# razoumov/radiativeTransfer

Hardware: AMD Instinct MI355X
Metric: cell·dir·ν updates/sec per iteration, 256³ grid; achieved HBM GB/s vs peak (higher is better)
Workload: dtype f64

## Files before the change

### radiativetransfer_amd/csrc/ftte_api.cpp

```cpp
#include "ftte_context.h"

using namespace ftte;

namespace ftte {

std::string g_create_error;

int fail(ftte_ctx *c, int code, const std::string &msg)
{
    if (c) c->err = msg;
    else g_create_error = msg;
    return code;
}

int check_single(ftte_ctx *c)
{
    if (c && c->multi) return check_ready(c, false);
    return c ? FTTE_OK : FTTE_ERR_ARG;
}

}


extern "C" {
// ... 288 lines not shown
    if (c->multi) return multi_counter(c, name);
    if (!std::strcmp(name, "devices")) return 1;
    if (!std::strcmp(name, "grid_builds")) return c->n_grid_builds;
    if (!std::strcmp(name, "plan_builds")) return c->n_plan_builds;
    if (!std::strcmp(name, "forest_builds")) return c->n_forest_builds;
    if (!std::strcmp(name, "device_objects")) return g_device_objects.load();
    if (!std::strcmp(name, "population_slots")) return c->point.tables.slot_count();
    if (!std::strcmp(name, "expansion_exact_tests")) return c->chem.expansion_tests;
    if (!std::strcmp(name, "medium_abun2")) return c->gas.ready_with_abundance(c->ncell) ? 1 : 0;
    if (!std::strcmp(name, "catalogue_stars")) return c->catalogue.stars();
    if (!std::strcmp(name, "catalogue_sources")) return c->catalogue.sources();
    if (!std::strncmp(name, "catalogue_ns_", 13)) {
        static const char *const phase[4] = {"locate", "count", "scan", "emit"};
        for (int p = 0; p < 4; ++p)
            if (!std::strcmp(name + 13, phase[p])) return catalogue_phase_ns(c->catalogue, p);
        return -1;
    }
    if (!std::strcmp(name, "hybrid_boxes")) return c->hplan.boxes();
    if (!std::strcmp(name, "hybrid_passes")) return c->hplan.passes();
    if (!std::strcmp(name, "fine_block")) return c->hplan.fine_block();
    if (!std::strcmp(name, "brick_form")) return c->last_brick_form;
    if (!std::strcmp(name, "brick_dataflow")) return c->last_brick_dataflow;
    if (!std::strcmp(name, "brick_whole")) return c->last_brick_whole;
    if (!std::strcmp(name, "nu_deal")) return c->opt.launch.nu_deal;
    if (!std::strcmp(name, "brick_chunk")) return c->bplan.valid ? c->bplan.chunk : 0;
    if (!std::strcmp(name, "brick_queue_mix")) return (c->bplan.valid && c->bplan.persistent) ? c->bplan.key.queue_mix : -1;
    if (!std::strcmp(name, "brick_groups")) return c->bplan.valid ? (long long)c->bplan.groups.size() : 0;
    if (!std::strcmp(name, "brick_accumulators")) return c->bplan.valid ? c->bplan.nacc[0] + c->bplan.nacc[1] + c->bplan.nacc[2] : 0;
    if (!std::strcmp(name, "brick_accumulators_0")) return c->bplan.valid ? c->bplan.nacc[0] : 0;
    if (!std::strcmp(name, "brick_accumulators_1")) return c->bplan.valid ? c->bplan.nacc[1] : 0;
    if (!std::strcmp(name, "brick_accumulators_2")) return c->bplan.valid ? c->bplan.nacc[2] : 0;
    if (!std::strcmp(name, "brick_stages")) return c->bplan.valid ? c->bplan.nstages : 0;
    if (!std::strcmp(name, "merge_points")) return c->bplan.valid ? (long long)c->bplan.merge_stage.size() : 0;
    if (!std::strcmp(name, "merge_blocks")) return c->bplan.valid ? (long long)c->bplan.merge_blocks.size() : 0;
    if (!std::strncmp(name, "merge_stage_", 12) || !std::strncmp(name, "merge_final_", 12)) {
        char *end = nullptr;
        const long k = std::strtol(name + 12, &end, 10);
        if (!c->bplan.valid || end == name + 12 || *end || k < 0 || k >= (long)c->bplan.merge_stage.size()) return -1;
        return name[6] == 's' ? c->bplan.merge_stage[(size_t)k] : (long long)c->bplan.merge_off[(size_t)k + 1];
    }
    return -1;
}

int ftte_launch_count(const ftte_ctx *c) { return !c ? 0 : c->multi ? multi_first(c)->timing_used : c->timing_used; }

int ftte_launch_info(ftte_ctx *c, int idx, double *ms, int64_t *updates)
// ... 335 lines not shown
```

### radiativetransfer_amd/csrc/ftte_brick.hip

```cpp
#include <hip/hip_runtime.h>

#include "ftte_internal.h"
#include "ftte_kernels.h"
#include "ftte_math.h"

namespace ftte {

using gcbyte = const __attribute__((address_space(1))) char;
using gbyte = __attribute__((address_space(1))) char;
using gcdouble = const __attribute__((address_space(1))) double;
using gdouble = __attribute__((address_space(1))) double;

__device__ __forceinline__ int uniform(int x) { return __builtin_amdgcn_readfirstlane(x); }
__device__ __forceinline__ gcbyte *lane_address(gcbyte *base, unsigned offset) { asm volatile("" : "+s"(base)); return base + offset; }
__device__ __forceinline__ gbyte *lane_address(gbyte *base, unsigned offset) { asm volatile("" : "+s"(base)); return base + offset; }
__device__ __forceinline__ unsigned here(unsigned offset) { asm volatile("" : "+v"(offset)); return offset; }
__device__ __forceinline__ long here(long step) { asm volatile("" : "+s"(step)); return step; }

template <int ROWS, bool NT>
__device__ __forceinline__ void load_rows(double (&dst)[ROWS], gcbyte *row, unsigned off, long step, int nrows)
{
    if (nrows == ROWS) {
        off = here(off);
#pragma unroll
// ... 663 lines not shown
                for (int r = 0; r < H; ++r) {
                    if (r < nrows) {
                        if (accumulate && atomic_acc) (void)__builtin_amdgcn_global_atomic_fadd_f64((gdouble *)lane_address(jrow, off), Jacc[r]);
                        else __builtin_nontemporal_store(Jacc[r], (gdouble *)lane_address(jrow, off));
                    }
                    jrow += rstep;
                }
            }
        }
        __syncthreads();
    }

    if (has_i_out) {
        for (int q = 0; q < ndir; ++q) {
            int d = p0 + q;
            d = d >= ndir ? d - ndir : d;
            gdouble *f = (gdouble *)(G->dir[d].faces + fnu);
#pragma unroll
            for (int r = 0; r < H; ++r) f[i_out + (long)r * up] = q ? state[((q - 1) * H + r) * 64 + lane] : cur[r];
        }
    }
}

__global__ void xcc_census_kernel(unsigned *mask)
{
    unsigned xcc;
    asm volatile("s_getreg_b32 %0, hwreg(HW_REG_XCC_ID)" : "=s"(xcc));
    if (threadIdx.x == 0) atomicOr(mask, 1u << (xcc & 15u));
}

int launch_xcc_census(unsigned *mask_dev, hipStream_t stream)
{
    hipLaunchKernelGGL(xcc_census_kernel, dim3(4096), dim3(64), 0, stream, mask_dev);
    return hipGetLastError() == hipSuccess ? 0 : -2;
}

int launch_brick_pair(const BrickLaunch &L, int max_dirs, int waves, int lds_pad, hipStream_t stream)
{
    if (L.ntasks <= 0) return 0;
    if (max_dirs < 1 || max_dirs > kBrickMaxDirs || L.ticket != nullptr) return -1;
    const dim3 grid((unsigned)L.ntasks * (unsigned)L.nnu);
    const size_t lds = ((size_t)(max_dirs - 1) * kBrickRows * 64 + 2 * max_dirs * 64) * sizeof(double) + (size_t)lds_pad;
    if (L.emit == 1) hipLaunchKernelGGL((brick_pair_kernel<3, 1>), grid, dim3(128), lds, stream, L, max_dirs);
    else if (L.emit == 2) hipLaunchKernelGGL((brick_pair_kernel<4, 2>), grid, dim3(128), lds, stream, L, max_dirs);
    else if (L.emit) return -1;
    else switch (waves) {
    case 2: hipLaunchKernelGGL((brick_pair_kernel<2, 0>), grid, dim3(128), lds, stream, L, max_dirs); break;
    case 3: hipLaunchKernelGGL((brick_pair_kernel<3, 0>), grid, dim3(128), lds, stream, L, max_dirs); break;
    case 4: hipLaunchKernelGGL((brick_pair_kernel<4, 0>), grid, dim3(128), lds, stream, L, max_dirs); break;
    default: return -1;
    }
    return hipGetLastError() == hipSuccess ? 0 : -2;
}

bool brick_whole_form(const BrickLaunch &L, int waves, bool masked)
{
    return !masked && !L.emit && !L.ticket && !L.queue && waves == 4 && L.n % 64 == 0 && L.n % kBrickRows == 0 && !L.atomic_acc && !L.ablate;
}

int launch_brick(const BrickLaunch &L, int max_dirs, int waves, int lds_pad, hipStream_t stream, bool masked, int persistent)
{
    if (L.ntasks <= 0) return 0;
    if (max_dirs < 1 || max_dirs > kBrickMaxDirs) return -1;
    if (L.tiled && (L.emit || masked)) return -1;
    const dim3 grid((unsigned)L.ntasks * (unsigned)L.nnu);
    const size_t lds = (size_t)(max_dirs - 1) * kBrickRows * 64 * sizeof(double) + (size_t)lds_pad;
    const bool flow = L.ticket != nullptr;
    if (L.queue) {
        if (masked || L.emit || !flow || persistent < 1) return -1;
        hipLaunchKernelGGL((brick_kernel<4, 0, 2>), dim3((unsigned)persistent), dim3(64), lds, stream, L);
        return hipGetLastError() == hipSuccess ? 0 : -2;
    }
    if (masked && !flow && L.emit) {
        if (L.emit == 1) hipLaunchKernelGGL((brick_kernel<2, 1, 0, true>), grid, dim3(64), lds, stream, L);
        else hipLaunchKernelGGL((brick_kernel<3, 2, 0, true>), grid, dim3(64), lds, stream, L);
        return hipGetLastError() == hipSuccess ? 0 : -2;
    }
    if (masked) {
        if (flow) return -1;
        hipLaunchKernelGGL((brick_kernel<3, 0, 0, true>), grid, dim3(64), lds, stream, L);
        return hipGetLastError() == hipSuccess ? 0 : -2;
    }
    if (L.emit == 1 && !flow) hipLaunchKernelGGL((brick_kernel<3, 1, 0>), grid, dim3(64), lds, stream, L);
    else if (L.emit == 2 && !flow) hipLaunchKernelGGL((brick_kernel<3, 2, 0>), grid, dim3(64), lds, stream, L);
    else if (L.emit) return -1;
// ... 15 lines not shown
```

### radiativetransfer_amd/csrc/ftte_bricks.h

```cpp
#pragma once

#include <algorithm>
#include <cstdio>
#include <cstdlib>
#include <cstring>
#include <functional>
#include <string>
#include <vector>

#include "../../include/ftte.h"
#include "ftte_device.h"
#include "ftte_internal.h"

namespace ftte {

struct DirPlan {
    int izone = 0, layout = 0;
    double phi = 0, theta = 0, w = 0;
    int64_t org = 0;
    int si = 0, sv = 0, su = 0;
    int u_lo = 1, v_lo = 1, ntu = 0, ntv = 0;
    int du_mid = 0, dv_mid = 0;
    size_t layer_off = 0;
    int slot = 0;
};

struct BrickKey {
    int n = 0;
    double box = 0;
    int chunk = 0, gmax = 0, share = 0;
    int want_dataflow = 0, want_glanes = 0;
    int nnu = 0, xcc_count = 0, queue_mix = 0;
    bool operator==(const BrickKey &o) const
    {
        return n == o.n && box == o.box && chunk == o.chunk && gmax == o.gmax && share == o.share && want_dataflow == o.want_dataflow &&
               want_glanes == o.want_glanes && nnu == o.nnu && xcc_count == o.xcc_count && queue_mix == o.queue_mix;
    }
};

struct BrickOptions {
    int chunk = 0, group = 0;
    int share = 2, team = -1, lanes = 2;
    int dataflow = 0;
    int queue_mix = 0;

    int brick_form(int nnu, int emit_mode) const { return team >= 0 ? team : (((nnu <= 4 || emit_mode) && !dataflow) ? 2 : 0); }

    BrickKey resolve(int n, int nnu, int emit_mode) const
    {
        BrickKey k;
        const int form = brick_form(nnu, emit_mode);
        k.n = n;
        k.chunk = std::min(chunk > 0 ? chunk : (nnu >= 4 ? 16 : nnu >= 2 ? 8 : 4), n);
        k.gmax = group > 0 ? group : (nnu >= 2 || form == 2 ? 3 : 2);
        k.share = share;
        k.want_dataflow = (dataflow && n % 64 == 0 && n % kBrickRows == 0 && n % k.chunk == 0 && form == 0 && !emit_mode) ? 1 : 0;
        k.want_glanes = k.want_dataflow ? 1 : (nnu >= lanes ? 1 : lanes);
        return k;
    }
    void persistent(BrickKey &k, int nnu, int xcc_count) const
    {
        if (!k.want_dataflow || dataflow != 3 || xcc_count < 1 || xcc_count > kBrickQueues) return;
        k.want_dataflow = 3; k.nnu = nnu; k.xcc_count = xcc_count; k.queue_mix = queue_mix;
    }
    BrickKey resolve_hybrid(int n, int nnu) const
    {
        BrickKey k;
        k.n = n;
        k.chunk = std::min(chunk > 0 ? chunk : 4, n);
        k.gmax = group > 0 ? group : (nnu >= 2 ? 3 : 2);
        k.share = share;
        return k;
    }
};

struct BrickPlan {
    bool valid = false;
    long long id = 0;
    BrickKey key;
    std::vector<double> phi, theta, w;
    int n = 0, chunk = 0;
    std::vector<DirPlan> dirs;
    std::vector<LayerRec> layers;
    struct Group { int izone = 0, layout = 0, acc = 0, offset = 0, lane = 0; std::vector<int> dirs; };
    std::vector<Group> groups;
    std::vector<BrickTask> tasks;
    bool dataflow = false;
    std::vector<int32_t> deps;
    bool persistent = false;
    std::vector<uint32_t> queue;
    uint32_t qoff[kBrickQueues] = {}, qlen[kBrickQueues] = {};
    int64_t qload[kBrickQueues] = {};
    int ut = kBrickRows, uw = 0;
    int64_t uqface_off = 0;
    int nslot = 2;
    int glanes = 1, nstages = 0;
    std::vector<size_t> stage_off;
    int64_t updates = 0;
    int ntu = 0, ntv = 0, nti = 0, up = 0, vp = 0, max_dirs = 0;
    int64_t face_elems = 0, vface_off = 0, iface_off = 0;
    int nacc[3] = {0, 0, 0};
    int nmb = 0;
    std::vector<int32_t> merge_blocks;
    std::vector<int> merge_stage;
    std::vector<size_t> merge_off;
};

struct SubGridPlan {
    int n = 0;
// ... 26 lines not shown
public:
    T *get() const { return buf_; }
    operator T *() const { return get(); }
    void reset() { buf_.reset(); held_.clear(); }
    hipError_t send(const T *src, size_t count)
    {
        bool fresh = false;
        hipError_t e = buf_.reserve(count, &fresh);
        if (fresh || e != hipSuccess) held_.clear();
        const size_t bytes = sizeof(T) * count;
        if (e != hipSuccess || !bytes || (held_.size() == bytes && !std::memcmp(held_.data(), src, bytes))) return e;
        held_.clear();
        if ((e = hipMemcpy(buf_, src, bytes, hipMemcpyHostToDevice)) == hipSuccess) held_.assign((const char *)src, (const char *)src + bytes);
        return e;
    }
private:
    DeviceBuffer<T> buf_;
    std::vector<char> held_;
};

struct BrickTables {
    DeviceBuffer<LayerRec> layers; DeviceBuffer<BrickTask> tasks; Sent<BrickGroup> groups;
    DeviceBuffer<int32_t> deps, merge_blocks; DeviceBuffer<uint32_t> queue;
    bool holds(const BrickPlan &P) const { return held_ != 0 && held_ == P.id; }
    hipError_t upload(const BrickPlan &P)
    {
        if (holds(P)) return hipSuccess;
        held_ = 0;
        hipError_t e;
        if ((e = to_device(layers, P.layers)) != hipSuccess || (e = to_device(tasks, P.tasks)) != hipSuccess) return e;
        if (P.dataflow && !P.deps.empty() && (e = to_device(deps, P.deps)) != hipSuccess) return e;
        if (!P.merge_blocks.empty() && (e = to_device(merge_blocks, P.merge_blocks)) != hipSuccess) return e;
        if (P.persistent && !P.queue.empty() && (e = to_device(queue, P.queue)) != hipSuccess) return e;
        held_ = P.id;
        return hipSuccess;
    }
private:
    long long held_ = 0;
};

inline BrickLaunch brick_launch(const BrickPlan &P, const BrickTables &T, size_t task0, size_t task1, int nu0, int nu1, int64_t group_stride,
                                int64_t face_stride, const double *uvb, int emit)
{
    BrickLaunch L;
    std::memset(&L, 0, sizeof L);
    L.groups = T.groups; L.tasks = T.tasks + task0; L.uvb = uvb;
    L.group_stride = group_stride; L.face_stride = face_stride;
    L.vface_off = P.vface_off; L.iface_off = P.iface_off; L.uqface_off = P.uqface_off;
    L.n = P.n; L.ntasks = (int)(task1 - task0); L.nnu = nu1 - nu0; L.nu0 = nu0; L.chunk = P.chunk;
    L.up = P.up; L.vp = P.vp; L.uw = P.uw; L.ut = P.ut; L.nslot = P.nslot;
    L.emit = emit; L.math = kMath;
    return L;
}

struct AccList { const double *acc[3 * kMaxAcc]; int layout[3 * kMaxAcc]; int count = 0; };
inline AccList acc_list(const DeviceBuffer<double> (&set)[3][kMaxAcc], const int (&nacc)[3], const int (&frame)[3], size_t offset = 0)
// ... 87 lines not shown
```

### radiativetransfer_amd/csrc/ftte_context.h

```cpp
#pragma once

#include <hip/hip_runtime_api.h>

#include <algorithm>
#include <cmath>
#include <cstdio>
#include <cstring>
#include <functional>
#include <string>
#include <vector>

#include "../../include/ftte.h"
#include "ftte_amr.h"
#include "ftte_analysis.h"
#include "ftte_bricks.h"
#include "ftte_gas.h"
#include "ftte_geometry.h"
#include "ftte_host.h"
#include "ftte_hybrid.h"
#include "ftte_kernels.h"
#include "ftte_lambda.h"
#include "ftte_medium.h"
#include "ftte_options.h"
#include "ftte_point.h"
// ... 22 lines not shown
namespace ftte { struct Multi; }

struct ftte_ctx {
    ftte::Multi *multi = nullptr;
    int device = 0;
    Stream stream;
    std::string err;

    bool grid_set = false;
    int n = 0;
    int64_t ncell = 0;
    double box = 0;

    Options opt;

    int nnu = 0;
    MediumField kappa;

    int emit_mode = 0;
    MediumField emis;

    DeviceBuffer<double> acc[3][kMaxAcc];

    int last_brick_form = -1, last_brick_dataflow = -1, last_brick_whole = 0;
    std::vector<Stream> lane_stream;
    std::vector<Event> pipe_up;
    std::vector<Event> lane_done;
    Event ev_fork;
    BrickDataflow bflow;
    int xcc_count = -1;
    int8_t xcc_queue[16] = {};
    long long brick_plans = 0;
    BrickPlan bplan;
    BrickTables btables;
    DeviceBuffer<double> d_faces;

    Plan plan;
    DeviceBuffer<LayerRec> d_layers;
    DeviceBuffer<WorkItem> d_items;
    Sent<double> d_uvb;
    bool plan_uploaded = false;

    std::vector<LaunchTiming> timing;
    int timing_used = 0;

    AmrTree tree;
    DeviceTree dtree;
// ... 118 lines not shown
```

### radiativetransfer_amd/csrc/ftte_internal.h

```cpp
#pragma once
#include <cstdint>

#include "ftte_math.h"

namespace ftte {

enum RayClass : int {
    RC_ONE = 0,
    RC_TWO_U = 1,
    RC_TWO_V = 2,
    RC_THREE_U = 3,
    RC_THREE_V = 4,
    RC_THREE_U_SWAP = 5,
    RC_THREE_V_SWAP = 6
};

struct LayerRec {
    double dpath[3];
    int32_t info;
    int32_t drift;
};
static_assert(sizeof(LayerRec) == 32, "LayerRec must be 32 bytes");

struct DirRec {
// ... 41 lines not shown
    const LayerRec *layers;
    double *faces;
    double w;
    double pad;
};

struct BrickGroup {
    BrickDir dir[kBrickMaxDirs];
    const double *kappa;
    const double *emis;
    double *J;
    int64_t org;
    int32_t si, sv, su;
    int32_t ndir;
    int32_t bu, bv;
    int64_t bi;
};

struct BrickTask { int16_t group, tu, tv, ti; };
constexpr int kBrickAccumulate = 0x4000;
constexpr int kBrickTuMask = 0x3ff, kBrickLaneLoShift = 10, kBrickGroupMask = 0xff, kBrickLaneHiShift = 8;
constexpr int kBrickTvMask = 0x3ff, kBrickBoxShift = 10, kBrickBoxMask = 31;
static_assert(sizeof(BrickTask) == 8, "BrickTask must be 8 bytes");

struct BrickLaunch {
    const BrickGroup *groups;
    const BrickTask *tasks;
    const double *uvb;
    int64_t group_stride;
    int64_t face_stride;
    int64_t vface_off, iface_off;
    int64_t uqface_off;
    int32_t n, ntasks, nnu, chunk;
    int32_t nu0;
    int32_t emit;
    int32_t up, vp;
    int32_t nslot;
    int32_t uw, ut;
    uint32_t *ticket, *done, *error;
    const int32_t *deps;
    uint32_t epoch;
    int32_t through;
    int32_t tiled, ablate;
    const uint32_t *queue;
    uint32_t qoff[kBrickQueues], qlen[kBrickQueues];
    int8_t xcc_queue[16];
    int32_t atomic_acc;
    int32_t sub;
    int32_t deal;
    ftte_consts math;
};

constexpr unsigned kXcds = 8;
struct BrickWork { unsigned task, slot; };
FTTE_HD BrickWork brick_deal(unsigned work, unsigned nnu, unsigned deal)
{
    BrickWork W;
    W.task = work / nnu;
    W.slot = work - W.task * nnu;
    if (deal) {
        const unsigned low = nnu & (0u - nnu), g = low < kXcds ? low : kXcds;
        W.slot = (W.slot + W.task / (kXcds / g * deal)) % nnu;
    }
    return W;
}

constexpr int kAmrBatch = 96;

struct SegRec {
    int32_t seg;
    int32_t up, up2;
    int32_t at;
// ... 91 lines not shown
```

### radiativetransfer_amd/csrc/ftte_kernels.h

```cpp
#pragma once
#include <hip/hip_runtime_api.h>

#include "ftte_internal.h"

namespace ftte {

int launch_sweep(const LaunchRec &L, int rows, int waves, int stack, int nnu, int lds_pad, hipStream_t stream);
int launch_brick(const BrickLaunch &L, int max_dirs, int waves, int lds_pad, hipStream_t stream, bool masked = false, int persistent = 0);
bool brick_whole_form(const BrickLaunch &L, int waves, bool masked = false);
int launch_xcc_census(unsigned *mask_dev, hipStream_t stream);
int launch_brick_pair(const BrickLaunch &L, int max_dirs, int waves, int lds_pad, hipStream_t stream);
int launch_to_layout(int layout, const double *src, double *dst, int n, int nnu, long group_stride, hipStream_t stream, bool tiled = false, int tchunk = 0);
int launch_set_layouts(const double *src, double *dst0, double *dst1, double *dst2, int n, int nnu, long group_stride, hipStream_t stream);
int launch_merge(const double *const *acc, const int *layout, int count, double *J, int n, int nnu, long group_stride,
                 bool accumulate, hipStream_t stream, const int32_t *leaf_of_base = nullptr, long j_stride = 0, bool tiled = false, int tchunk = 0);
int launch_merge_blocks(const double *const *acc, const int *layout, int count, double *J, int n, int nnu, long group_stride,
                        const int32_t *blocks, int nblocks, int nmb, hipStream_t stream, bool tiled = false, int tchunk = 0);
int launch_sum_parts(const double *const *parts, int nparts, double *out, long count, hipStream_t stream);
int launch_base_cells(const double *leaf_values, const int32_t *leaf_of_base, double *base_values, long nbase, long ncell, int nnu,
                      hipStream_t stream);
int launch_amr_export(const AmrLevelRec &A, int64_t most_exports, hipStream_t stream);
int launch_amr_fine_import(const AmrLevelRec &A, int64_t most_imports, hipStream_t stream);
int launch_opacity(const double *HI, const double *HeI, const double *HeII, const double *beta, double *kappa, long ncell,
                   int nnu, hipStream_t stream);

int launch_cell_major(const double *src, double *dst, long ncell, int nnu, hipStream_t stream, const int32_t *cells = nullptr, long count = 0);
int launch_amr_level(const AmrLevelRec &A, hipStream_t stream);
int launch_amr_levels(const AmrLevelRec &A, const int64_t *tables, int ndepth, hipStream_t stream);
int launch_amr_combine(const AmrLevelRec &A, double *J, bool zero_first, hipStream_t stream);

int launch_rate_table(const FreqBin *bins, int nbins, int npop, double *tables, double *logtab, hipStream_t stream);
// ... 15 lines not shown
```

### radiativetransfer_amd/csrc/ftte_options.h

```cpp
#pragma once

#include <cstring>
#include <string>

#include "ftte_bricks.h"
#include "ftte_hybrid.h"
#include "ftte_tiles.h"

namespace ftte {

struct TileOptions { int rows = 8, slots = 8, waves = 4, stack = 1; };

struct LaunchOptions {
    int brick_waves = 4, pair_waves = 4;
    int atomic_acc = 0;
    int nu_deal = 16;
    int ablate = 0;
    int tiled = 0;
    int merge_overlap = 1;
    int forest_fuse = 4096;
    int lds_pad = 0;
};

struct RouteOptions { int engine = 0, forest = 0; };

struct Options {
    BrickOptions brick;
    HybridOptions hybrid;
    TileOptions tile;
    LaunchOptions launch;
    RouteOptions route;
};

struct OptionRow {
    const char *name;
    int lo, hi;
    bool (*also)(int);
    const char *refusal;
    int &(*at)(Options &);
    bool invalidates;
};

inline bool power_of_two(int v) { return (v & (v - 1)) == 0; }
inline bool not_one(int v) { return v != 1; }
// ... 54 lines not shown
```

### radiativetransfer_amd/csrc/ftte_plan.cpp

```cpp
#include "ftte_context.h"

namespace ftte {

int build_plan(ftte_ctx *c, int rows, int stack, int ndir, const double *phi, const double *theta, const double *w)
{
    Plan &P = c->plan;
    if (P.valid && P.n == c->n && P.rows == rows && P.slots == c->opt.tile.slots && P.stack == stack && P.box == c->box && same_list(P.phi, phi, ndir) &&
        same_list(P.theta, theta, ndir) && same_list(P.w, w, ndir))
        return FTTE_OK;
    ++c->n_plan_builds;
    c->plan_uploaded = false;
    std::string why;
    const int rc = plan_tiles(TileInputs{c->n, c->box, rows, stack, c->opt.tile.slots, ndir, phi, theta, w}, P, &why);
    return rc ? fail(c, rc, why) : FTTE_OK;
}

int build_brick_plan(ftte_ctx *c, int ndir, const double *phi, const double *theta, const double *w)
{
    BrickPlan &P = c->bplan;
    BrickKey key = c->opt.brick.resolve(c->n, c->nnu, c->emit_mode);
    key.box = c->box;
    if (key.want_dataflow && c->opt.brick.dataflow == 3) {
        const int rc = xcc_census(c);
        if (rc) return rc;
        c->opt.brick.persistent(key, c->nnu, c->xcc_count);
    }
    if (P.valid && P.key == key && same_list(P.phi, phi, ndir) && same_list(P.theta, theta, ndir) && same_list(P.w, w, ndir)) return FTTE_OK;
    ++c->n_plan_builds;
    const long long id = ++c->brick_plans;
    std::string why;
    const int rc = plan_bricks(BrickInputs{key, ndir, phi, theta, w}, P, &why);
    P.id = id;
    return rc ? fail(c, rc, why) : FTTE_OK;
}

}
```

### radiativetransfer_amd/csrc/ftte_planner.cpp

```cpp
#include <algorithm>
#include <cmath>
#include <cstdio>
#include <cstring>
#include <thread>

#include "ftte_geometry.h"
#include "ftte_hybrid.h"
#include "ftte_tiles.h"

namespace ftte {

static int fail(std::string *err, int code, const std::string &msg)
{
    if (err) *err = msg;
    return code;
}

int plan_direction(int n_grid, double box, int d, double phi_d, double theta_d, double w_d, int tile_rows, std::vector<ftte_pattern> &pat,
                   std::vector<int> &du_cum, std::vector<int> &dv_cum, DirPlan &D, LayerRec *layers_of_d, size_t layer_off,
                   const SubGridPlan *sub, std::string *err)
{
    const int n = sub ? sub->n : n_grid;
    const double cell = sub ? sub->cell : box / (double)n;
    const long nn = (long)n * n;
// ... 205 lines not shown
    P.tasks.resize(off[nlists]);
    std::vector<size_t> fill(off.begin(), off.end() - 1);
    for (size_t g : order) {
        const BrickPlan::Group &G = P.groups[g];
        const std::vector<size_t> &F = first[(size_t)G.layout * kMaxAcc + G.acc];
        visit(g, [&](size_t list, size_t launch, int tu, int tv, int ti, BrickTask T) {
            if (launch > F[brick_index(P, G, tu, tv, ti)]) T.ti = (int16_t)(T.ti | kBrickAccumulate);
            P.tasks[fill[list]++] = T;
        });
    }
    return off;
}


void deal_group_lanes(BrickPlan &P, int want_glanes)
{
    P.glanes = std::max(1, std::min(want_glanes, P.nacc[0] + P.nacc[1] + P.nacc[2]));
    int next = 0;
    std::vector<int> lane_of(3 * (size_t)kMaxAcc, -1);
    for (auto &G : P.groups) {
        int &l = lane_of[(size_t)G.layout * kMaxAcc + G.acc];
        if (l < 0) l = next++ % P.glanes;
        G.lane = l;
    }
}

void write_stage_lists(BrickPlan &P, int ndir)
{
    int max_offset = 0;
    for (const auto &G : P.groups) max_offset = std::max(max_offset, G.offset);
    const size_t nstages = P.groups.empty() ? 0 : (size_t)(P.ntu + P.ntv + P.nti - 2 + max_offset);
    P.nstages = (int)nstages;
    const std::vector<size_t> off = build_task_lists(P, largest_groups_first(P), (size_t)P.glanes * nstages, [&](size_t g, auto put) {
        const BrickPlan::Group &G = P.groups[g];
        for_each_brick(P, [&](int tu, int tv, int ti) {
            const size_t st = (size_t)(tu + tv + ti + G.offset);
            put((size_t)G.lane * nstages + st, st, tu, tv, ti, BrickTask{(int16_t)g, (int16_t)tu, (int16_t)tv, (int16_t)ti});
        });
    });
    P.stage_off.resize((size_t)P.glanes * (nstages + 1));
    for (size_t l = 0; l < (size_t)P.glanes; ++l)
        for (size_t st = 0; st <= nstages; ++st) P.stage_off[l * (nstages + 1) + st] = off[l * nstages + st];
    P.updates = (int64_t)P.n * P.n * P.n * ndir;
}

int link_dependencies(BrickPlan &P, std::string *err)
// ... 113 lines not shown
    std::vector<std::vector<uint32_t>> lists((size_t)nq);
    for (size_t t = 0; t < P.tasks.size(); ++t) {
        const BrickPlan::Group &G = P.groups[(size_t)P.tasks[t].group];
        const size_t a = (size_t)G.layout * kMaxAcc + G.acc;
        for (int nu = 0; nu < nnu; ++nu)
            lists[(size_t)queue_of[(size_t)nu * acc_dirs.size() + a]].push_back((uint32_t)(t * (size_t)nnu + (size_t)nu));
    }
    for (int q = 0; q < kBrickQueues; ++q) {
        P.qoff[q] = (uint32_t)P.queue.size();
        P.qlen[q] = q < nq ? (uint32_t)lists[(size_t)q].size() : 0;
        P.qload[q] = q < nq ? load[q] * n * n * n : 0;
        if (q < nq) P.queue.insert(P.queue.end(), lists[(size_t)q].begin(), lists[(size_t)q].end());
    }
}

}

int plan_bricks(const BrickInputs &in, BrickPlan &P, std::string *err)
{
    const BrickKey &K = in.key;
    int rc;
    if ((rc = plan_brick_groups(P, K.n, K.box, in.ndir, in.phi, in.theta, in.w, K.chunk, K.gmax, K.share, K.want_dataflow, false, nullptr, err))) return rc;
    P.key = K;
    deal_group_lanes(P, K.want_glanes);
    write_stage_lists(P, in.ndir);
    if (P.dataflow && !P.tasks.empty() && (rc = link_dependencies(P, err))) return rc;
    if (!P.dataflow && P.glanes == 1 && !P.tasks.empty()) cut_merge_points(P);
    if (P.dataflow && K.want_dataflow == 3 && !P.tasks.empty()) deal_queues(P, K.nnu, K.xcc_count, K.queue_mix);
    P.valid = true;
    return FTTE_OK;
}

int plan_tiles(const TileInputs &in, Plan &P, std::string *err)
{
    const int n = in.n, slots = in.slots, ndir = in.ndir;
    const int tile_rows = in.stack * in.rows - 1;
    P = Plan();
    P.n = n; P.rows = in.rows; P.slots = slots; P.stack = in.stack; P.box = in.box;
    P.phi.assign(in.phi, in.phi + ndir); P.theta.assign(in.theta, in.theta + ndir); P.w.assign(in.w, in.w + ndir);
    P.dirs.resize(ndir);
    P.layers.resize((size_t)ndir * n);

    std::vector<ftte_pattern> pat(n);
    std::vector<int> du_cum(n + 1), dv_cum(n + 1);
    int in_layout[3] = {0, 0, 0};

    for (int d = 0; d < ndir; ++d) {
        DirPlan &D = P.dirs[d];
// ... 610 lines not shown
```

### radiativetransfer_amd/csrc/ftte_sweeps.cpp

```cpp
#include "ftte_context.h"

namespace ftte {

int ensure_kappa(ftte_ctx *c, int nnu)
{
    const size_t need = (size_t)nnu * c->ncell;
    if (nnu != c->nnu) c->emit_mode = 0;
    if (c->kappa.source() && c->kappa.capacity() >= need) return FTTE_OK;
    c->emis.release(); c->emit_mode = 0;
    FTTE_HIP(c, c->kappa.reserve_source(need));
    return FTTE_OK;
}

int ensure_timing(ftte_ctx *c, size_t count)
{
    while (c->timing.size() < count) {
        LaunchTiming t;
        FTTE_HIP(c, t.start.create());
        FTTE_HIP(c, t.stop.create());
        c->timing.push_back(std::move(t));
    }
    return FTTE_OK;
}

// ... 438 lines not shown
    FTTE_HIP(c, ensure_lanes(c->lane_stream, c->lane_done, (size_t)nlanes - 1));
    FTTE_HIP(c, c->ev_fork.create(hipEventDisableTiming));
    overlap = O.merge_overlap && !lane_ends && !P.dataflow && P.glanes == 1 && !P.groups.empty() && !P.merge_stage.empty();
    npoints = overlap ? P.merge_stage.size() : 0;
    FTTE_HIP(c, ensure_events(c->ev_merge_point, (size_t)nlanes * npoints, hipEventDisableTiming));
    if ((rc = ensure_timing(c, 1))) return rc;
    c->timing_used = 0;
    return FTTE_OK;
}

int BrickSweep::one_launch()
{
    BrickLaunch L = launch(0, P.tasks.size(), 0, nnu);
    FTTE_HIP(c, c->bflow.prepare(L, c->btables, P.tasks.size() * (size_t)nnu, stream));
    L.through = c->opt.brick.dataflow == 2 ? 1 : 0;
    int persistent = 0;
    if (P.persistent) {
        L.queue = c->btables.queue;
        std::memcpy(L.qoff, P.qoff, sizeof L.qoff); std::memcpy(L.qlen, P.qlen, sizeof L.qlen); std::memcpy(L.xcc_queue, c->xcc_queue, sizeof L.xcc_queue);
        hipDeviceProp_t prop;
        FTTE_HIP(c, hipGetDeviceProperties(&prop, c->device));
        persistent = (int)std::min<size_t>((size_t)prop.multiProcessorCount * 16, P.queue.size());
    }
    c->last_brick_form = 0; c->last_brick_dataflow = P.persistent ? 3 : c->opt.brick.dataflow == 2 ? 2 : 1; c->last_brick_whole = 0;
    const int lrc = launch_brick(L, P.max_dirs, O.brick_waves, O.lds_pad, stream, false, persistent);
    if (lrc) return fail(c, lrc == -1 ? FTTE_ERR_ARG : FTTE_ERR_NO_DEVICE, "brick kernel launch failed");
    FTTE_HIP(c, c->bflow.read_back(P, stream));
    return FTTE_OK;
}

int BrickSweep::lane_stages(int lane, LaunchTiming &T)
{
    const size_t nstages = (size_t)P.nstages;
    int rc;
    hipStream_t q = queue(lane);
    if (lane) FTTE_HIP(c, hipStreamWaitEvent(q, c->ev_fork, 0));
    const LaneSlice S = slice(lane);
    const size_t *off = &P.stage_off[(size_t)(P.glanes > 1 ? lane : 0) * (nstages + 1)];
    if (pipe) {
        FTTE_HIP(c, ensure_events(c->pipe_up, (size_t)nlanes, hipEventDisableTiming));
        if (lane) FTTE_HIP(c, hipStreamWaitEvent(q, c->pipe_up[(size_t)lane - 1], 0));
        if ((rc = upload_on(c, q, c->kappa.source() + S.first, pipe->kappa + S.first, S.bytes))) return rc;
        FTTE_HIP(c, hipEventRecord(c->pipe_up[(size_t)lane], q));
    }
    if (lane_ends) {
        for (int l = 1; l < 3; ++l)
            if (lane_layout[l] && launch_to_layout(l, c->kappa.source() + S.first, c->kappa.in_layout(l) + S.first, n, S.nu1 - S.nu0, (long)c->ncell, q))
                return fail(c, FTTE_ERR_NO_DEVICE, "layout kernel launch failed");
        FTTE_HIP(c, hipEventRecord(T.first[(size_t)lane], q));
    }
    for (size_t st = 0, mp = 0; st < nstages; ++st) {
        if (off[st + 1] != off[st]) {
            const BrickLaunch L = launch(off[st], off[st + 1], S.nu0, S.nu1);
            const int form = c->opt.brick.brick_form(nnu, c->emit_mode);
            c->last_brick_form = form; c->last_brick_dataflow = 0; c->last_brick_whole = form != 2 && brick_whole_form(L, O.brick_waves);
            const int lrc = form == 2 ? launch_brick_pair(L, P.max_dirs, O.pair_waves, O.lds_pad, q) : launch_brick(L, P.max_dirs, O.brick_waves, O.lds_pad, q);
            if (lrc) return fail(c, lrc == -1 ? FTTE_ERR_ARG : FTTE_ERR_NO_DEVICE, "brick kernel launch failed");
        }
        if (overlap && mp < npoints && (size_t)P.merge_stage[mp] == st) {
            FTTE_HIP(c, hipEventRecord(c->ev_merge_point[(size_t)lane * npoints + mp], q));
            ++mp;
        }
    }
    if (lane_ends) {
        FTTE_HIP(c, hipEventRecord(T.last[(size_t)lane], q));
        const AccList A = acc_list(c->acc, P.nacc, frame, S.first);
        if (launch_merge(A.acc, A.layout, A.count, J_dev + S.first, n, S.nu1 - S.nu0, (long)c->ncell, false, q, nullptr, 0, tiled, tchunk))
            return fail(c, FTTE_ERR_NO_DEVICE, "merge kernel launch failed");
        if (pipe && is_registered(c, pipe->J + S.first, S.bytes))
            FTTE_HIP(c, hipMemcpyAsync(pipe->J + S.first, J_dev + S.first, S.bytes, hipMemcpyDeviceToHost, q));
    }
    if (lane) {
        FTTE_HIP(c, hipEventRecord(c->lane_done[(size_t)lane - 1], q));
        FTTE_HIP(c, hipStreamWaitEvent(stream, c->lane_done[(size_t)lane - 1], 0));
    }
// ... 185 lines not shown
```

Measured before the change: 425.1 billion.

## Pair sibling brick groups into two-wave duo blocks sharing J accumulation

Adds a duo brick kernel in which two 64-lane waves in one 128-thread block each sweep a different direction group over the same brick, or two unrelated lone tasks. For linked pairs the helper wave hands its J contribution to the owner through LDS, and only the owner reads and writes J. The planner links adjacent groups that share an izone and layout into owner/helper seats, which cuts the number of J accumulator passes and global J read-modify-writes. The cost is twice the LDS per block, two barriers per layer, and possible load imbalance when the paired groups have different direction counts.

```diff
diff --git a/radiativetransfer_amd/csrc/ftte_api.cpp b/radiativetransfer_amd/csrc/ftte_api.cpp
--- a/radiativetransfer_amd/csrc/ftte_api.cpp
+++ b/radiativetransfer_amd/csrc/ftte_api.cpp
@@ -334,6 +334,7 @@
     if (!std::strcmp(name, "brick_form")) return c->last_brick_form;
     if (!std::strcmp(name, "brick_dataflow")) return c->last_brick_dataflow;
     if (!std::strcmp(name, "brick_whole")) return c->last_brick_whole;
+    if (!std::strcmp(name, "brick_duo")) return c->last_brick_duo;
     if (!std::strcmp(name, "nu_deal")) return c->opt.launch.nu_deal;
     if (!std::strcmp(name, "brick_chunk")) return c->bplan.valid ? c->bplan.chunk : 0;
     if (!std::strcmp(name, "brick_queue_mix")) return (c->bplan.valid && c->bplan.persistent) ? c->bplan.key.queue_mix : -1;
diff --git a/radiativetransfer_amd/csrc/ftte_brick.hip b/radiativetransfer_amd/csrc/ftte_brick.hip
--- a/radiativetransfer_amd/csrc/ftte_brick.hip
+++ b/radiativetransfer_amd/csrc/ftte_brick.hip
@@ -709,6 +709,178 @@
     }
 }
 
+__global__ void __launch_bounds__(128, 4) brick_duo_kernel(const BrickLaunch L, int max_dirs)
+{
+    extern __shared__ double duo_lds[];
+    constexpr int R = kBrickRows;
+    using cgroup = const __attribute__((address_space(4))) BrickGroup;
+    using clayer = const __attribute__((address_space(4))) LayerRec;
+    const int lane = threadIdx.x & 63;
+    const int wv = uniform((int)(threadIdx.x >> 6));
+    const int nnu = L.nnu;
+    const BrickWork W = brick_deal(blockIdx.x, (unsigned)nnu, (unsigned)L.deal);
+    const int nu = L.nu0 + (int)W.slot;
+    const __attribute__((address_space(4))) unsigned long *seat = (const __attribute__((address_space(4))) unsigned long *)(unsigned long)L.seats + 2ul * W.task;
+    const unsigned long raw0 = seat[0], raw1 = seat[1];
+    const int linked = (uniform((int)(raw0 >> 48)) / kBrickLinked) & 1;
+    const int helper = linked & wv;
+    const unsigned long raw = wv ? raw1 : raw0, where = linked ? raw0 : raw;
+    const int group = uniform((int)(int16_t)(raw & 0xffffu));
+    if (group < 0) return;
+    const int tu = uniform((int)(int16_t)((where >> 16) & 0xffffu)), tv = uniform((int)(int16_t)((where >> 32) & 0xffffu));
+    const int ti_field = uniform((int)(int16_t)(where >> 48));
+    const int ti = ti_field & (kBrickLinked - 1);
+    const int accumulate = (ti_field / kBrickAccumulate) & 1 & (helper ^ 1);
+    const int shift = wv * (max_dirs - 1) * R * 64;
+    const int lx = lane + shift;
+    double *state = duo_lds + R * 64;
+    cgroup *G = (cgroup *)(L.groups + group);
+    const int n = L.n, chunk = L.chunk, up = L.up, vp = L.vp;
+    const int ndir = G->ndir;
+    const double uvb = ((const __attribute__((address_space(4))) double *)(unsigned long)L.uvb)[nu];
+    double lead = L.math.c[9];
+    asm volatile("" : "+v"(lead));
+
+    const int sv = G->sv, si = G->si;
+    const bool mirror_u = G->su < 0;
+    const long org = G->org;
+    gcbyte *kbase = (gcbyte *)(G->kappa + (long)nu * L.group_stride + org);
+    gbyte *jbase = (gbyte *)(G->J + (long)nu * L.group_stride + org);
+
+    const int cu = 64 * tu + lane + 1;
+    const int cv0 = R * tv + 1;
+    const unsigned off0 = 8u * (unsigned)(mirror_u ? n + 1 - cu : cu);
+    const long row_bytes = 8l * sv;
+    const int i0 = ti * chunk + 1, i1 = i0 + chunk - 1;
+    const bool has_u_in = tu > 0, has_u_out = 64 * (tu + 1) < n;
+    const bool has_v_in = tv > 0, has_v_out = R * (tv + 1) < n;
+    const bool has_i_in = ti > 0, has_i_out = i1 < n;
+    const long fnu = (long)nu * L.face_stride;
+    const int uw = L.uw, ut = L.ut;
+    const int ns = L.nslot, sl = ti % ns;
+    const long u_out = ((long)(tu * ns + sl) * chunk) * uw + ut * tv;
+    const long u_in = ((long)((tu > 0 ? tu - 1 : 0) * ns + sl) * chunk) * uw + ut * tv;
+    const long v_out = L.vface_off + ((long)(tv * ns + sl) * chunk) * up + 64 * tu;
+    const long v_in = L.vface_off + ((long)((tv > 0 ? tv - 1 : 0) * ns + sl) * chunk) * up + 64 * tu;
+    const long i_in = L.iface_off + ((long)sl * vp + R * tv) * up + 64 * tu + lane;
+
+    int p0 = (ndir - (i0 - 1) % ndir) % ndir;
+    double kap_next[R], kap_odd[R], cur[R];
+    const long row0 = cv0 * row_bytes;
+    load_rows<R, false>(kap_next, kbase + 8l * i0 * si + row0, off0, row_bytes, R);
+    gcdouble *uvb_at = (gcdouble *)L.uvb + nu;
+    asm volatile("" : "+s"(uvb_at));
+    const long ist = has_i_in ? (long)up : 0l;
+    {
+        gcdouble *f = has_i_in ? (gcdouble *)(G->dir[p0].faces + fnu) + i_in : uvb_at;
+#pragma unroll
+        for (int r = 0; r < R; ++r) cur[r] = f[r * ist];
+    }
+    for (int k = 0; k + 1 < ndir; ++k) {
+        int d = p0 + 1 + k;
+        d = d >= ndir ? d - ndir : d;
+        gcdouble *f = has_i_in ? (gcdouble *)(G->dir[d].faces + fnu) + i_in : uvb_at;
+        double parked[R];
+#pragma unroll
+        for (int r = 0; r < R; ++r) parked[r] = f[r * ist];
+        __builtin_amdgcn_sched_barrier(0);
+#pragma unroll
+        for (int r = 0; r < R; ++r) state[(k * R + r) * 64 + lx] = parked[r];
+    }
+#pragma unroll
+    for (int r = 0; r < R; ++r) asm volatile("" ::"v"(kap_next[r]), "v"(cur[r]));
+    auto layer = [&](const int i, const double(&kap)[R], double(&kn)[R]) __attribute__((always_inline)) {
+        const int il = i - i0;
+        const double xs[1] = {0.0};
+        double Jacc[R];
+        gbyte *jplane = jbase + 8l * i * si;
+        const long rstep = here(row_bytes);
+        int adds = accumulate, pair = linked, helps = helper;
+        asm volatile("" : "+s"(adds), "+s"(pair), "+s"(helps));
+        if (adds) load_rows<R, true>(Jacc, (gcbyte *)jplane + row0, off0, rstep, R);
+        else {
+#pragma unroll
+            for (int r = 0; r < R; ++r) Jacc[r] = 0.0;
+        }
+        load_rows<R, false>(kn, kbase + 8l * (i < i1 ? i + 1 : i) * si + row0, off0, rstep, R);
+        for (int j = 0; j < ndir; ++j) {
+            int d = p0 + j;
+            d = d >= ndir ? d - ndir : d;
+            if (j) {
+#pragma unroll
+                for (int r = 0; r < R; ++r) {
+                    const double parked = state[((j - 1) * R + r) * 64 + lx];
+                    state[((j - 1) * R + r) * 64 + lx] = cur[r];
+                    cur[r] = parked;
+                }
+            }
+            clayer *rp = (clayer *)(G->dir[d].layers) + (i - 1);
+            const double d0 = rp->dpath[0], d1 = rp->dpath[1], d2 = rp->dpath[2];
+            const int rc = rp->info & 7;
+            const double w = G->dir[d].w;
+            gbyte *f = (gbyte *)(G->dir[d].faces + fnu);
+            gcbyte *uin = has_u_in ? (gcbyte *)f + 8 * (u_in + (long)il * uw) : nullptr;
+            gbyte *uout = has_u_out ? f + 8 * (u_out + (long)il * uw) : nullptr;
+            gcbyte *vin = has_v_in ? (gcbyte *)f + 8 * (v_in + (long)il * up - shift) : nullptr;
+            gbyte *vout = has_v_out ? f + 8 * (v_out + (long)il * up - shift) : nullptr;
+            gcbyte *vb = (gcbyte *)uvb_at;
+            const bool third_first = rc == RC_THREE_U_SWAP || rc == RC_THREE_V_SWAP;
+            switch (rc) {
+            case RC_ONE: brick_step<RC_ONE, 0, R, true>(L.math, lead, cur, kap, xs, Jacc, false, d0, d1, d2, w, uvb, uin, uout, vin, vout, lx, false, false, 0, 63 + shift, true, nullptr, nullptr, vb); break;
+            case RC_TWO_U: brick_step<RC_TWO_U, 0, R, true>(L.math, lead, cur, kap, xs, Jacc, false, d0, d1, d2, w, uvb, uin, uout, vin, vout, lx, false, false, 0, 63 + shift, true, nullptr, nullptr, vb); break;
+            case RC_TWO_V: brick_step<RC_TWO_V, 0, R, true>(L.math, lead, cur, kap, xs, Jacc, false, d0, d1, d2, w, uvb, uin, uout, vin, vout, lx, false, false, 0, 63 + shift, true, nullptr, nullptr, vb); break;
+            case RC_THREE_U:
+            case RC_THREE_U_SWAP:
+                brick_step<RC_THREE_U, 0, R, true>(L.math, lead, cur, kap, xs, Jacc, third_first, d0, d1, d2, w, uvb, uin, uout, vin, vout, lx, false, false, 0, 63 + shift, true, nullptr, nullptr, vb);
+                break;
+            default:
+                brick_step<RC_THREE_V, 0, R, true>(L.math, lead, cur, kap, xs, Jacc, third_first, d0, d1, d2, w, uvb, uin, uout, vin, vout, lx, false, false, 0, 63 + shift, true, nullptr, nullptr, vb);
+                break;
+            }
+        }
+        p0 = p0 ? p0 - 1 : ndir - 1;
+        if (pair) {
+            asm volatile("s_waitcnt lgkmcnt(0)\n\ts_barrier" ::: "memory");
+            double *rows = duo_lds + ((int)here((unsigned)lx) - shift);
+            if (helps) {
+#pragma unroll
+                for (int r = 0; r < R; ++r) rows[r * 64] = Jacc[r];
+            }
+            asm volatile("s_waitcnt lgkmcnt(0)\n\ts_barrier" ::: "memory");
+            if (!helps) {
+#pragma unroll
+                for (int r = 0; r < R; ++r) Jacc[r] += rows[r * 64];
+            }
+        }
+        if (!helps) {
+            gbyte *jrow = jplane + row0;
+            const unsigned off = here(off0);
+#pragma unroll
+            for (int r = 0; r < R; ++r) {
+                __builtin_nontemporal_store(Jacc[r], (gdouble *)lane_address(jrow, off));
+                jrow += rstep;
+            }
+        }
+    };
+    for (int i = i0;; i += 2) {
+        layer(i, kap_next, kap_odd);
+        if (i == i1) break;
+        layer(i + 1, kap_odd, kap_next);
+        if (i + 1 == i1) break;
+    }
+
+    if (has_i_out) {
+        const long i_out = L.iface_off + ((long)((ti + 1) % ns) * vp + R * tv) * up + 64 * tu + ((int)here((unsigned)lx) - shift);
+        for (int j = 0; j < ndir; ++j) {
+            int d = p0 + j;
+            d = d >= ndir ? d - ndir : d;
+            gdouble *f = (gdouble *)(G->dir[d].faces + fnu);
+#pragma unroll
+            for (int r = 0; r < R; ++r) f[i_out + (long)r * up] = j ? state[((j - 1) * R + r) * 64 + lx] : cur[r];
+        }
+    }
+}
+
 __global__ void xcc_census_kernel(unsigned *mask)
 {
     unsigned xcc;
@@ -740,6 +912,16 @@
     return hipGetLastError() == hipSuccess ? 0 : -2;
 }
 
+int launch_brick_duo(const BrickLaunch &L, int max_dirs, int lds_pad, hipStream_t stream)
+{
+    if (L.ntasks <= 0) return 0;
+    if (max_dirs < 1 || max_dirs > kBrickMaxDirs || !L.seats || lds_pad < 0) return -1;
+    if (L.emit || L.ticket || L.queue || L.tiled || L.atomic_acc || L.ablate || L.sub || L.n % 64 || L.n % kBrickRows || L.n % L.chunk) return -1;
+    const dim3 grid((unsigned)L.ntasks * (unsigned)L.nnu);
+    hipLaunchKernelGGL(brick_duo_kernel, grid, dim3(128), brick_duo_lds(max_dirs, lds_pad), stream, L, max_dirs);
+    return hipGetLastError() == hipSuccess ? 0 : -2;
+}
+
 bool brick_whole_form(const BrickLaunch &L, int waves, bool masked)
 {
     return !masked && !L.emit && !L.ticket && !L.queue && waves == 4 && L.n % 64 == 0 && L.n % kBrickRows == 0 && !L.atomic_acc && !L.ablate;
@@ -748,6 +930,7 @@
 int launch_brick(const BrickLaunch &L, int max_dirs, int waves, int lds_pad, hipStream_t stream, bool masked, int persistent)
 {
     if (L.ntasks <= 0) return 0;
+    if (L.seats) return masked || persistent || waves != 4 ? -1 : launch_brick_duo(L, max_dirs, lds_pad, stream);
     if (max_dirs < 1 || max_dirs > kBrickMaxDirs) return -1;
     if (L.tiled && (L.emit || masked)) return -1;
     const dim3 grid((unsigned)L.ntasks * (unsigned)L.nnu);
diff --git a/radiativetransfer_amd/csrc/ftte_bricks.h b/radiativetransfer_amd/csrc/ftte_bricks.h
--- a/radiativetransfer_amd/csrc/ftte_bricks.h
+++ b/radiativetransfer_amd/csrc/ftte_bricks.h
@@ -31,10 +31,11 @@
     int chunk = 0, gmax = 0, share = 0;
     int want_dataflow = 0, want_glanes = 0;
     int nnu = 0, xcc_count = 0, queue_mix = 0;
+    int duo = 0;
     bool operator==(const BrickKey &o) const
     {
         return n == o.n && box == o.box && chunk == o.chunk && gmax == o.gmax && share == o.share && want_dataflow == o.want_dataflow &&
-               want_glanes == o.want_glanes && nnu == o.nnu && xcc_count == o.xcc_count && queue_mix == o.queue_mix;
+               want_glanes == o.want_glanes && nnu == o.nnu && xcc_count == o.xcc_count && queue_mix == o.queue_mix && duo == o.duo;
     }
 };
 
@@ -63,6 +64,12 @@
         if (!k.want_dataflow || dataflow != 3 || xcc_count < 1 || xcc_count > kBrickQueues) return;
         k.want_dataflow = 3; k.nnu = nnu; k.xcc_count = xcc_count; k.queue_mix = queue_mix;
     }
+    void visits(BrickKey &k, int nnu, int emit_mode, bool plain_launch) const
+    {
+        if (brick_form(nnu, emit_mode) != 0 || emit_mode || k.want_dataflow || k.share < 1 || !plain_launch) return;
+        if (k.n % 64 || k.n % kBrickRows || k.n % k.chunk || k.n / k.chunk >= kBrickLinked) return;
+        k.duo = 1;
+    }
     BrickKey resolve_hybrid(int n, int nnu) const
     {
         BrickKey k;
@@ -82,9 +89,13 @@
     int n = 0, chunk = 0;
     std::vector<DirPlan> dirs;
     std::vector<LayerRec> layers;
-    struct Group { int izone = 0, layout = 0, acc = 0, offset = 0, lane = 0; std::vector<int> dirs; };
+    struct Group { int izone = 0, layout = 0, acc = 0, offset = 0, lane = 0; std::vector<int> dirs; int partner = -1; bool helper = false; };
     std::vector<Group> groups;
     std::vector<BrickTask> tasks;
+    bool duo = false;
+    std::vector<BrickSeat> seats;
+    std::vector<size_t> seat_off;
+    int nvisits = 0, nlinked = 0;
     bool dataflow = false;
     std::vector<int32_t> deps;
     bool persistent = false;
@@ -157,6 +168,7 @@
 struct BrickTables {
     DeviceBuffer<LayerRec> layers; DeviceBuffer<BrickTask> tasks; Sent<BrickGroup> groups;
     DeviceBuffer<int32_t> deps, merge_blocks; DeviceBuffer<uint32_t> queue;
+    DeviceBuffer<BrickSeat> seats;
     bool holds(const BrickPlan &P) const { return held_ != 0 && held_ == P.id; }
     hipError_t upload(const BrickPlan &P)
     {
@@ -167,6 +179,7 @@
         if (P.dataflow && !P.deps.empty() && (e = to_device(deps, P.deps)) != hipSuccess) return e;
         if (!P.merge_blocks.empty() && (e = to_device(merge_blocks, P.merge_blocks)) != hipSuccess) return e;
         if (P.persistent && !P.queue.empty() && (e = to_device(queue, P.queue)) != hipSuccess) return e;
+        if (P.duo && (e = to_device(seats, P.seats)) != hipSuccess) return e;
         held_ = P.id;
         return hipSuccess;
     }
diff --git a/radiativetransfer_amd/csrc/ftte_context.h b/radiativetransfer_amd/csrc/ftte_context.h
--- a/radiativetransfer_amd/csrc/ftte_context.h
+++ b/radiativetransfer_amd/csrc/ftte_context.h
@@ -68,7 +68,7 @@
 
     DeviceBuffer<double> acc[3][kMaxAcc];
 
-    int last_brick_form = -1, last_brick_dataflow = -1, last_brick_whole = 0;
+    int last_brick_form = -1, last_brick_dataflow = -1, last_brick_whole = 0, last_brick_duo = 0;
     std::vector<Stream> lane_stream;
     std::vector<Event> pipe_up;
     std::vector<Event> lane_done;
diff --git a/radiativetransfer_amd/csrc/ftte_internal.h b/radiativetransfer_amd/csrc/ftte_internal.h
--- a/radiativetransfer_amd/csrc/ftte_internal.h
+++ b/radiativetransfer_amd/csrc/ftte_internal.h
@@ -1,4 +1,5 @@
 #pragma once
+#include <cstddef>
 #include <cstdint>
 
 #include "ftte_math.h"
@@ -87,6 +88,10 @@
 constexpr int kBrickTuMask = 0x3ff, kBrickLaneLoShift = 10, kBrickGroupMask = 0xff, kBrickLaneHiShift = 8;
 constexpr int kBrickTvMask = 0x3ff, kBrickBoxShift = 10, kBrickBoxMask = 31;
 static_assert(sizeof(BrickTask) == 8, "BrickTask must be 8 bytes");
+struct BrickSeat { BrickTask place[2]; };
+constexpr int kBrickLinked = 0x2000;
+static_assert(sizeof(BrickSeat) == 16, "BrickSeat must be 16 bytes");
+constexpr size_t brick_duo_lds(int max_dirs, int lds_pad) { return (size_t)lds_pad + 2 * (size_t)(max_dirs - 1) * kBrickRows * 64 * 8 + (size_t)kBrickRows * 64 * 8; }
 
 struct BrickLaunch {
     const BrickGroup *groups;
@@ -113,6 +118,7 @@
     int32_t atomic_acc;
     int32_t sub;
     int32_t deal;
+    const BrickSeat *seats;
     ftte_consts math;
 };
 
diff --git a/radiativetransfer_amd/csrc/ftte_kernels.h b/radiativetransfer_amd/csrc/ftte_kernels.h
--- a/radiativetransfer_amd/csrc/ftte_kernels.h
+++ b/radiativetransfer_amd/csrc/ftte_kernels.h
@@ -7,6 +7,7 @@
 
 int launch_sweep(const LaunchRec &L, int rows, int waves, int stack, int nnu, int lds_pad, hipStream_t stream);
 int launch_brick(const BrickLaunch &L, int max_dirs, int waves, int lds_pad, hipStream_t stream, bool masked = false, int persistent = 0);
+int launch_brick_duo(const BrickLaunch &L, int max_dirs, int lds_pad, hipStream_t stream);
 bool brick_whole_form(const BrickLaunch &L, int waves, bool masked = false);
 int launch_xcc_census(unsigned *mask_dev, hipStream_t stream);
 int launch_brick_pair(const BrickLaunch &L, int max_dirs, int waves, int lds_pad, hipStream_t stream);
diff --git a/radiativetransfer_amd/csrc/ftte_options.h b/radiativetransfer_amd/csrc/ftte_options.h
--- a/radiativetransfer_amd/csrc/ftte_options.h
+++ b/radiativetransfer_amd/csrc/ftte_options.h
@@ -20,6 +20,7 @@
     int merge_overlap = 1;
     int forest_fuse = 4096;
     int lds_pad = 0;
+    bool plain() const { return brick_waves == 4 && !atomic_acc && !ablate && !tiled; }
 };
 
 struct RouteOptions { int engine = 0, forest = 0; };
diff --git a/radiativetransfer_amd/csrc/ftte_plan.cpp b/radiativetransfer_amd/csrc/ftte_plan.cpp
--- a/radiativetransfer_amd/csrc/ftte_plan.cpp
+++ b/radiativetransfer_amd/csrc/ftte_plan.cpp
@@ -25,6 +25,8 @@
         if (rc) return rc;
         c->opt.brick.persistent(key, c->nnu, c->xcc_count);
     }
+    c->opt.brick.visits(key, c->nnu, c->emit_mode, c->opt.launch.plain());
+
     if (P.valid && P.key == key && same_list(P.phi, phi, ndir) && same_list(P.theta, theta, ndir) && same_list(P.w, w, ndir)) return FTTE_OK;
     ++c->n_plan_builds;
     const long long id = ++c->brick_plans;
diff --git a/radiativetransfer_amd/csrc/ftte_planner.cpp b/radiativetransfer_amd/csrc/ftte_planner.cpp
--- a/radiativetransfer_amd/csrc/ftte_planner.cpp
+++ b/radiativetransfer_amd/csrc/ftte_planner.cpp
@@ -251,6 +251,68 @@
         int &l = lane_of[(size_t)G.layout * kMaxAcc + G.acc];
         if (l < 0) l = next++ % P.glanes;
         G.lane = l;
+    }
+}
+
+void link_visits(BrickPlan &P)
+{
+    const size_t ng = P.groups.size();
+    for (size_t g0 = 0, g1; g0 < ng; g0 = g1) {
+        for (g1 = g0 + 1; g1 < ng && P.groups[g1].izone == P.groups[g0].izone && P.groups[g1].layout == P.groups[g0].layout; ++g1) {}
+        if (g1 - g0 >= 2) P.duo = true;
+    }
+    P.nvisits = (int)ng;
+    if (!P.duo) return;
+    P.nvisits = 0;
+    for (size_t g0 = 0, g1; g0 < ng; g0 = g1) {
+        for (g1 = g0 + 1; g1 < ng && P.groups[g1].izone == P.groups[g0].izone && P.groups[g1].layout == P.groups[g0].layout; ++g1) {}
+        const int step = g1 - g0 >= 2 ? P.groups[g0 + 1].offset - P.groups[g0].offset : 1;
+        for (size_t g = g0; g < g1; ++g) {
+            BrickPlan::Group &G = P.groups[g];
+            const size_t p = g - g0;
+            G.offset = (int)(p / 2) * step;
+            G.helper = p % 2 == 1;
+            G.partner = G.helper ? (int)g - 1 : g + 1 < g1 ? (int)g + 1 : -1;
+            if (!G.helper) ++P.nvisits;
+        }
+    }
+}
+
+void seat_stage_lists(BrickPlan &P)
+{
+    const size_t nb = (size_t)P.ntu * P.ntv * P.nti;
+    const size_t none = ~(size_t)0;
+    std::vector<size_t> helper_at(P.groups.size() * nb, none);
+    for (size_t q = 0; q < P.tasks.size(); ++q) {
+        BrickTask &T = P.tasks[q];
+        if (!P.groups[(size_t)T.group].helper) continue;
+        T.ti = (int16_t)(T.ti & ~kBrickAccumulate);
+        helper_at[(size_t)T.group * nb + brick_index(P, T.tu, T.tv, T.ti)] = q;
+    }
+    auto ndirs = [&](const BrickTask &T) { return T.group < 0 ? (size_t)0 : P.groups[(size_t)T.group].dirs.size(); };
+    const BrickTask empty{-1, 0, 0, 0};
+    P.seat_off.assign((size_t)P.glanes * ((size_t)P.nstages + 1), 0);
+    for (size_t l = 0; l < (size_t)P.glanes; ++l) {
+        for (size_t st = 0; st < (size_t)P.nstages; ++st) {
+            const size_t q0 = P.stage_off[l * ((size_t)P.nstages + 1) + st], q1 = P.stage_off[l * ((size_t)P.nstages + 1) + st + 1];
+            std::vector<BrickSeat> seats;
+            std::vector<BrickTask> lone;
+            for (size_t q = q0; q < q1; ++q) {
+                const BrickTask &T = P.tasks[q];
+                const BrickPlan::Group &G = P.groups[(size_t)T.group];
+                if (G.helper) continue;
+                if (G.partner < 0) { lone.push_back(T); continue; }
+                BrickTask own = T, help = P.tasks[helper_at[(size_t)G.partner * nb + brick_index(P, T.tu, T.tv, T.ti & (kBrickAccumulate - 1))]];
+                own.ti = (int16_t)(own.ti | kBrickLinked); help.ti = (int16_t)(help.ti | kBrickLinked);
+                seats.push_back(BrickSeat{{own, help}});
+                ++P.nlinked;
+            }
+            for (size_t k = 0; k < lone.size(); k += 2) seats.push_back(BrickSeat{{lone[k], k + 1 < lone.size() ? lone[k + 1] : empty}});
+            std::stable_sort(seats.begin(), seats.end(), [&](const BrickSeat &x, const BrickSeat &y) { return ndirs(x.place[0]) + ndirs(x.place[1]) > ndirs(y.place[0]) + ndirs(y.place[1]); });
+            P.seats.insert(P.seats.end(), seats.begin(), seats.end());
+            P.seat_off[l * ((size_t)P.nstages + 1) + st + 1] = P.seats.size();
+        }
+        if (l + 1 < (size_t)P.glanes) P.seat_off[(l + 1) * ((size_t)P.nstages + 1)] = P.seats.size();
     }
 }
 
@@ -410,8 +472,11 @@
     int rc;
     if ((rc = plan_brick_groups(P, K.n, K.box, in.ndir, in.phi, in.theta, in.w, K.chunk, K.gmax, K.share, K.want_dataflow, false, nullptr, err))) return rc;
     P.key = K;
+    P.nvisits = (int)P.groups.size();
+    if (K.duo) link_visits(P);
     deal_group_lanes(P, K.want_glanes);
     write_stage_lists(P, in.ndir);
+    if (P.duo) seat_stage_lists(P);
     if (P.dataflow && !P.tasks.empty() && (rc = link_dependencies(P, err))) return rc;
     if (!P.dataflow && P.glanes == 1 && !P.tasks.empty()) cut_merge_points(P);
     if (P.dataflow && K.want_dataflow == 3 && !P.tasks.empty()) deal_queues(P, K.nnu, K.xcc_count, K.queue_mix);
diff --git a/radiativetransfer_amd/csrc/ftte_sweeps.cpp b/radiativetransfer_amd/csrc/ftte_sweeps.cpp
--- a/radiativetransfer_amd/csrc/ftte_sweeps.cpp
+++ b/radiativetransfer_amd/csrc/ftte_sweeps.cpp
@@ -484,7 +484,7 @@
         FTTE_HIP(c, hipGetDeviceProperties(&prop, c->device));
         persistent = (int)std::min<size_t>((size_t)prop.multiProcessorCount * 16, P.queue.size());
     }
-    c->last_brick_form = 0; c->last_brick_dataflow = P.persistent ? 3 : c->opt.brick.dataflow == 2 ? 2 : 1; c->last_brick_whole = 0;
+    c->last_brick_form = 0; c->last_brick_dataflow = P.persistent ? 3 : c->opt.brick.dataflow == 2 ? 2 : 1; c->last_brick_whole = 0; c->last_brick_duo = 0;
     const int lrc = launch_brick(L, P.max_dirs, O.brick_waves, O.lds_pad, stream, false, persistent);
     if (lrc) return fail(c, lrc == -1 ? FTTE_ERR_ARG : FTTE_ERR_NO_DEVICE, "brick kernel launch failed");
     FTTE_HIP(c, c->bflow.read_back(P, stream));
@@ -511,8 +511,16 @@
                 return fail(c, FTTE_ERR_NO_DEVICE, "layout kernel launch failed");
         FTTE_HIP(c, hipEventRecord(T.first[(size_t)lane], q));
     }
+    const size_t *seat_off = P.duo ? &P.seat_off[(size_t)(P.glanes > 1 ? lane : 0) * (nstages + 1)] : nullptr;
     for (size_t st = 0, mp = 0; st < nstages; ++st) {
-        if (off[st + 1] != off[st]) {
+        if (P.duo && seat_off[st + 1] != seat_off[st]) {
+            BrickLaunch L = launch(off[st], off[st + 1], S.nu0, S.nu1);
+            L.seats = c->btables.seats + seat_off[st]; L.ntasks = (int)(seat_off[st + 1] - seat_off[st]);
+            c->last_brick_form = 0; c->last_brick_dataflow = 0; c->last_brick_whole = 1; c->last_brick_duo = P.nlinked;
+            const int lrc = launch_brick(L, P.max_dirs, O.brick_waves, O.lds_pad, q);
+            if (lrc) return fail(c, lrc == -1 ? FTTE_ERR_ARG : FTTE_ERR_NO_DEVICE, "brick kernel launch failed");
+        } else if (!P.duo && off[st + 1] != off[st]) {
+            c->last_brick_duo = 0;
             const BrickLaunch L = launch(off[st], off[st + 1], S.nu0, S.nu1);
             const int form = c->opt.brick.brick_form(nnu, c->emit_mode);
             c->last_brick_form = form; c->last_brick_dataflow = 0; c->last_brick_whole = form != 2 && brick_whole_form(L, O.brick_waves);
```

New measurement: 454.1 billion, median of 6. 6.8% higher.
